# qinzheng93/GeoTransformer

Hardware: NVIDIA H100
Metric: point-cloud pairs/sec (3DMatch-shape synth) (higher is better)
Workload: dtype f32

## Files before the change

geotransformer_b200/csrc/evaluation.cu:

```cuda
#include "common.cuh"
#include "geob200.h"

namespace geob200 {

__device__ __forceinline__ float sqn3(float x, float y, float z) { return __fadd_rn(__fadd_rn(__fmul_rn(x, x), __fmul_rn(y, y)), __fmul_rn(z, z)); }
__device__ __forceinline__ float sqd_mm(float ax, float ay, float az, float a2, float bx, float by, float bz, float b2) {
    const float xy = fmaf(az, bz, fmaf(ay, by, __fmul_rn(ax, bx)));
    return fmaxf(__fadd_rn(__fsub_rn(a2, __fmul_rn(2.0f, xy)), b2), 0.0f);
}
__device__ __forceinline__ void xform(const float* T, float x, float y, float z, float& ox, float& oy, float& oz) {
    ox = fmaf(z, T[2], fmaf(y, T[1], x * T[0])) + T[3];
    oy = fmaf(z, T[6], fmaf(y, T[5], x * T[4])) + T[7];
    oz = fmaf(z, T[10], fmaf(y, T[9], x * T[8])) + T[11];
}

__global__ void __launch_bounds__(256) nc_prepare_kernel(const float* __restrict__ ref_nodes, const float* __restrict__ src_nodes,
                                                         const float* __restrict__ ref_knn_pts, const float* __restrict__ src_knn_pts,
                                                         const unsigned char* __restrict__ ref_knn_masks,
                                                         const unsigned char* __restrict__ src_knn_masks, const __grid_constant__ Segs cl,
                                                         int B, int K, const float* __restrict__ T, float* __restrict__ nodes_out,
                                                         float* __restrict__ pts_out, float* __restrict__ max_dist, int* __restrict__ n_valid) {
    const int lane = threadIdx.x & 31;
    const int s = blockIdx.y;
    const int m = blockIdx.x * 8 + (threadIdx.x >> 5);
    if (m >= cl.count[s]) return;
    const bool src = s >= B;
    const float* __restrict__ nodes = src ? src_nodes : ref_nodes;
    const float* __restrict__ knn_pts = src ? src_knn_pts : ref_knn_pts;
    const unsigned char* __restrict__ knn_masks = src ? src_knn_masks : ref_knn_masks;
    {
        const long long r = cl.start[s], r_in = src ? r - cl.start[B] : r;
        nodes += 3 * r_in; knn_pts += 3 * r_in * K; nodes_out += 3 * r; pts_out += 3 * r * K; max_dist += r; n_valid += r;
        if (knn_masks != nullptr) knn_masks += r_in * K;
        T = (T != nullptr && src) ? T + 16 * (s - B) : nullptr;
    }
    float nx = nodes[3 * m], ny = nodes[3 * m + 1], nz = nodes[3 * m + 2];
    if (T != nullptr) xform(T, nx, ny, nz, nx, ny, nz);
    float md = 0.f;
    int nv = 0;
    for (int i = lane; i < K; i += 32) {
        const float* p = knn_pts + ((long long)m * K + i) * 3;
        float px = p[0], py = p[1], pz = p[2];
        if (T != nullptr) xform(T, px, py, pz, px, py, pz);
        float* o = pts_out + ((long long)m * K + i) * 3;
        o[0] = px; o[1] = py; o[2] = pz;
        const bool ok = knn_masks == nullptr || knn_masks[(long long)m * K + i];
        const float dx = px - nx, dy = py - ny, dz = pz - nz;
        if (ok) { md = fmaxf(md, sqrtf(sqn3(dx, dy, dz))); ++nv; }
    }
    md = warp_max(md);
#pragma unroll
    for (int o = 16; o > 0; o >>= 1) nv += __shfl_xor_sync(0xffffffffu, nv, o);
    if (lane == 0) {
        nodes_out[3 * m] = nx; nodes_out[3 * m + 1] = ny; nodes_out[3 * m + 2] = nz;
        max_dist[m] = md;
        n_valid[m] = nv;
    }
}

__global__ void __launch_bounds__(256) nc_overlap_kernel(const float* __restrict__ ref_nodes, const float* __restrict__ src_nodes,
                                                         const float* __restrict__ ref_pts, const float* __restrict__ src_pts,
                                                         const unsigned char* __restrict__ ref_knn_masks,
                                                         const unsigned char* __restrict__ src_knn_masks,
                                                         const unsigned char* __restrict__ ref_masks, const unsigned char* __restrict__ src_masks,
                                                         const float* __restrict__ ref_max, const float* __restrict__ src_max,
                                                         const int* __restrict__ ref_nv, const int* __restrict__ src_nv,
                                                         const __grid_constant__ Segs R, const __grid_constant__ Segs Q,
                                                         const __grid_constant__ Segs NN, int K, float pos_radius,
                                                         float* __restrict__ overlap ) {
    const int b = blockIdx.y;
    const int M = R.count[b], N = Q.count[b];
    if ((int)blockIdx.x >= M) return;
    {
        const long long r = R.start[b], q = Q.start[b];
        ref_nodes += 3 * r; ref_pts += 3 * r * K; ref_max += r; ref_nv += r;
        if (ref_knn_masks != nullptr) ref_knn_masks += r * K;
        if (ref_masks != nullptr) ref_masks += r;
        src_nodes += 3 * q; src_pts += 3 * q * K; src_max += q; src_nv += q;
        if (src_knn_masks != nullptr) src_knn_masks += q * K;
        if (src_masks != nullptr) src_masks += q;
        overlap += NN.start[b];
    }
    extern __shared__ float sm[];
    float4* rp = reinterpret_cast<float4*>(sm);
    float4* sp = rp + K;
    int* rhit = reinterpret_cast<int*>(sp + K);
    int* shit = rhit + K;
    __shared__ int tot[2];
    const int m = blockIdx.x;
    const float r2 = pos_radius * pos_radius;
    for (int i = threadIdx.x; i < K; i += blockDim.x) {
        const float* p = ref_pts + ((long long)m * K + i) * 3;
        const bool ok = ref_knn_masks == nullptr || ref_knn_masks[(long long)m * K + i];
        rp[i] = make_float4(p[0], p[1], p[2], ok ? sqn3(p[0], p[1], p[2]) : -1.f);
    }
    const bool m_ok = ref_masks == nullptr || ref_masks[m];
    const float mx = ref_nodes[3 * m], my = ref_nodes[3 * m + 1], mz = ref_nodes[3 * m + 2];
    const float m2 = sqn3(mx, my, mz);
    __syncthreads();
    for (int n = 0; n < N; ++n) {
        float ov = 0.f;
        const bool n_ok = src_masks == nullptr || src_masks[n];
        const float sx = src_nodes[3 * n], sy = src_nodes[3 * n + 1], sz = src_nodes[3 * n + 2];
        const float dist = sqrtf(sqd_mm(mx, my, mz, m2, sx, sy, sz, sqn3(sx, sy, sz)));
        const bool inter = m_ok && n_ok && (ref_max[m] + src_max[n] + pos_radius - dist > 0.f);
        if (inter) {
            for (int j = threadIdx.x; j < K; j += blockDim.x) {
                const float* p = src_pts + ((long long)n * K + j) * 3;
                const bool ok = src_knn_masks == nullptr || src_knn_masks[(long long)n * K + j];
                sp[j] = make_float4(p[0], p[1], p[2], ok ? sqn3(p[0], p[1], p[2]) : -1.f);
                shit[j] = 0;
                rhit[j] = 0;
            }
            __syncthreads();
            for (int e = threadIdx.x; e < K * K; e += blockDim.x) {
                const int i = e / K, j = e % K;
                const float4 a = rp[i], b = sp[j];
                if (a.w >= 0.f && b.w >= 0.f && sqd_mm(a.x, a.y, a.z, a.w, b.x, b.y, b.z, b.w) < r2) { rhit[i] = 1; shit[j] = 1; }
            }
            __syncthreads();
            int cr = 0, cs = 0;
            for (int i = threadIdx.x; i < K; i += blockDim.x) { cr += rhit[i]; cs += shit[i]; }
            if (threadIdx.x == 0) { tot[0] = 0; tot[1] = 0; }
            __syncthreads();
            if (cr) atomicAdd(&tot[0], cr);
            if (cs) atomicAdd(&tot[1], cs);
            __syncthreads();
            ov = ((float)tot[0] / (float)ref_nv[m] + (float)tot[1] / (float)src_nv[n]) / 2.0f;
            __syncthreads();
        }
        if (threadIdx.x == 0) overlap[(long long)m * N + n] = ov;
    }
}

__global__ void __launch_bounds__(1024) nc_compact_kernel(const float* __restrict__ overlap, const __grid_constant__ Segs R,
                                                          const __grid_constant__ Segs Q, const __grid_constant__ Segs NN,
                                                          long long* __restrict__ idx, float* __restrict__ ov_out, int* __restrict__ count) {
    const int b = blockIdx.x;
    const int M = R.count[b], N = Q.count[b];
    overlap += NN.start[b]; idx += 2ll * NN.start[b]; ov_out += NN.start[b]; count += b;
    __shared__ int warp_tot[32];
    __shared__ int carry;
    const int lane = threadIdx.x & 31, warp = threadIdx.x >> 5;
    if (threadIdx.x == 0) carry = 0;
    __syncthreads();
    const long long total = (long long)M * N;
    for (long long base = 0; base < total; base += 4096) {
        const long long t0 = base + 4ll * threadIdx.x;
        float v[4];
        int f = 0;
#pragma unroll
        for (int u = 0; u < 4; ++u) {
            v[u] = (t0 + u < total) ? overlap[t0 + u] : 0.f;
            f += v[u] > 0.f ? 1 : 0;
        }
        int incl = f;
#pragma unroll
        for (int o = 1; o < 32; o <<= 1) {
            const int y = __shfl_up_sync(0xffffffffu, incl, o);
            if (lane >= o) incl += y;
        }
        if (lane == 31) warp_tot[warp] = incl;
        __syncthreads();
        int off = carry + incl - f;
        for (int w = 0; w < warp; ++w) off += warp_tot[w];
#pragma unroll
        for (int u = 0; u < 4; ++u)
            if (v[u] > 0.f) {
                idx[2ll * off] = (t0 + u) / N;
                idx[2ll * off + 1] = (t0 + u) % N;
                ov_out[off] = v[u];
                ++off;
            }
        __syncthreads();
        if (threadIdx.x == 0) { int s = 0; for (int w = 0; w < 32; ++w) s += warp_tot[w]; carry += s; }
        __syncthreads();
    }
    if (threadIdx.x == 0) *count = carry;
}

__global__ void __launch_bounds__(1024) evaluate_kernel(const long long* __restrict__ gt_idx, const float* __restrict__ gt_ov,
                                                        const __grid_constant__ Segs G, float acc_overlap,
                                                        const long long* __restrict__ ref_corr_idx, const long long* __restrict__ src_corr_idx,
                                                        int n_node_corr, const float* __restrict__ ref_corr_pts,
                                                        const float* __restrict__ src_corr_pts, int n_corr, float acc_radius,
                                                        const float* __restrict__ T_gt, const float* __restrict__ T_est, int t_ld,
                                                        const float* __restrict__ src_points, const __grid_constant__ Segs S0, int mode,
                                                        float acc_rmse, float acc_rre, float acc_rte, float* __restrict__ metrics, int m_ld,
                                                        const int* __restrict__ n_gt_dev, const int* __restrict__ n_node_corr_dev,
                                                        const int* __restrict__ n_corr_dev) {
    const int b = blockIdx.x;
    int n_gt = G.count[b];
    gt_idx += 2ll * G.start[b]; gt_ov += G.start[b];
    ref_corr_idx += (long long)b * n_node_corr; src_corr_idx += (long long)b * n_node_corr;
    ref_corr_pts += 3ll * b * n_corr; src_corr_pts += 3ll * b * n_corr;
    T_gt += 16 * b; T_est += (long long)b * t_ld;
    src_points += 3ll * S0.start[b];
    const int n_src = S0.count[b];
    metrics += (long long)b * m_ld;
    if (n_gt_dev != nullptr) n_gt_dev += b;
    if (n_node_corr_dev != nullptr) n_node_corr_dev += b;
    if (n_corr_dev != nullptr) n_corr_dev += b;
    if (n_gt_dev != nullptr) n_gt = *n_gt_dev;
    if (n_node_corr_dev != nullptr) n_node_corr = min(n_node_corr, *n_node_corr_dev);
    if (n_corr_dev != nullptr) n_corr = *n_corr_dev;
    __shared__ double red[32];
    __shared__ float Tg[16], Te[16], Tr[16];
    const int lane = threadIdx.x & 31, warp = threadIdx.x >> 5;
    if (threadIdx.x < 16) { Tg[threadIdx.x] = T_gt[threadIdx.x]; Te[threadIdx.x] = T_est[threadIdx.x]; }
    __syncthreads();
    auto block_sum = [&](double v) -> double {
        v = warp_sum_d(v);
        __syncthreads();
        if (lane == 0) red[warp] = v;
        __syncthreads();
        double s = 0.0;
        for (int w = 0; w < (int)(blockDim.x >> 5); ++w) s += red[w];
        return s;
    };
    const double nan = __longlong_as_double(0x7ff8000000000000LL);
    double hit = 0.0;
    for (int c = warp; c < n_node_corr; c += (int)(blockDim.x >> 5)) {
        const long long r = ref_corr_idx[c], s = src_corr_idx[c];
        int found = 0;
        for (int g = lane; g < n_gt; g += 32)
            if (gt_idx[2ll * g] == r && gt_idx[2ll * g + 1] == s && gt_ov[g] > acc_overlap) found = 1;
        found = __any_sync(0xffffffffu, found);
        if (lane == 0) hit += found;
    }
    const double hits = block_sum(hit);
    const double pir = n_node_corr > 0 ? hits / n_node_corr : nan;
    double inl = 0.0;
    for (int c = threadIdx.x; c < n_corr; c += blockDim.x) {
        float x, y, z;
        xform(Tg, src_corr_pts[3ll * c], src_corr_pts[3ll * c + 1], src_corr_pts[3ll * c + 2], x, y, z);
        const float dx = ref_corr_pts[3ll * c] - x, dy = ref_corr_pts[3ll * c + 1] - y, dz = ref_corr_pts[3ll * c + 2] - z;
        inl += (sqrtf(sqn3(dx, dy, dz)) < acc_radius) ? 1.0 : 0.0;
    }
    const double inls = block_sum(inl);
    const double ir = n_corr > 0 ? inls / n_corr : nan;
    if (threadIdx.x == 0) {
        for (int i = 0; i < 3; ++i) {
            for (int j = 0; j < 3; ++j) {
                double a = 0.0;
                for (int k = 0; k < 3; ++k) a += (double)Tg[4 * k + i] * Te[4 * k + j];
                Tr[4 * i + j] = (float)a;
            }
            double b = 0.0;
            for (int k = 0; k < 3; ++k) b += (double)Tg[4 * k + i] * ((double)Te[4 * k + 3] - Tg[4 * k + 3]);
            Tr[4 * i + 3] = (float)b;
        }
    }
    __syncthreads();
    double se = 0.0;
    if (mode != 1) {
        for (int p = threadIdx.x; p < n_src; p += blockDim.x) {
            const float px = src_points[3ll * p], py = src_points[3ll * p + 1], pz = src_points[3ll * p + 2];
            float x, y, z, gx = px, gy = py, gz = pz;
            if (mode == 0) {
                xform(Tr, px, py, pz, x, y, z);
            } else {
                xform(Te, px, py, pz, x, y, z);
                xform(Tg, px, py, pz, gx, gy, gz);
            }
            se += sqrtf(sqn3(x - gx, y - gy, z - gz));
        }
    }
    const double ses = block_sum(se);
    const double rmse = mode == 1 ? nan : (n_src > 0 ? ses / n_src : nan);
    if (threadIdx.x == 0) {
        float tr = 0.f;
        for (int i = 0; i < 3; ++i) {
            float d = 0.f;
            for (int k = 0; k < 3; ++k) d = fmaf(Te[4 * k + i], Tg[4 * k + i], d);
            tr += d;
        }
        float x = 0.5f * (tr - 1.0f);
        x = fminf(fmaxf(x, -1.0f), 1.0f);
        const float rre = 180.0f * acosf(x) / 3.14159265358979323846f;
        const float dtx = Tg[3] - Te[3], dty = Tg[7] - Te[7], dtz = Tg[11] - Te[11];
        const float rte = sqrtf(sqn3(dtx, dty, dtz));
        metrics[0] = (float)pir;
        metrics[1] = (float)ir;
        metrics[2] = rre;
// ... 197 lines not shown
        float s = 0.f;
        for (int k = 0; k < n; ++k) s += G[side ? (long long)k * N + line : (long long)line * N + k] * other[(long long)k * C + c];
        out[c] = s;
    }
}

__global__ void __launch_bounds__(32) closs_finalize_kernel(const float* __restrict__ ell_r, const unsigned char* __restrict__ kept_r,
                                                            const float* __restrict__ ell_c, const unsigned char* __restrict__ kept_c,
                                                            const __grid_constant__ Segs R, const __grid_constant__ Segs Q,
                                                            float* __restrict__ out, long long ld) {
    const int p = blockIdx.x, lane = threadIdx.x;
    double m[2];
    for (int side = 0; side < 2; ++side) {
        const float* ell = side ? ell_c : ell_r;
        const unsigned char* kept = side ? kept_c : kept_r;
        const int s0 = side ? Q.start[p] : R.start[p], n = side ? Q.count[p] : R.count[p];
        double s = 0.0, k = 0.0;
        for (int i = lane; i < n; i += 32)
            if (kept[s0 + i]) { s += ell[s0 + i]; k += 1.0; }
        s = warp_sum_d(s);
        k = warp_sum_d(k);
        m[side] = (float)(s / k);
    }
    if (lane == 0) out[p * ld + 1] = __fdiv_rn(__fadd_rn((float)m[0], (float)m[1]), 2.0f);
}

template <int K, int MODE>
__global__ void __launch_bounds__(256) floss_patch_kernel(const float* __restrict__ ref_pts, const float* __restrict__ src_pts,
                                                          const unsigned char* __restrict__ ref_masks,
                                                          const unsigned char* __restrict__ src_masks, float* __restrict__ scores,
                                                          const float* __restrict__ T, int P, const int* __restrict__ count, float r2,
                                                          double* __restrict__ psum, int* __restrict__ pcnt, const float* __restrict__ grad,
                                                          long long gld, int with_w, float w_f) {
    __shared__ float4 rp[K], sp[K];
    __shared__ int rhit[K], shit[K];
    __shared__ double redd[8];
    __shared__ int redi[8];
    __shared__ float Tm[16];
    const int p = blockIdx.y, q = blockIdx.x;
    const long long patch = (long long)p * P + q;
    const bool live = count == nullptr || q < count[p];
    if (threadIdx.x < 16) Tm[threadIdx.x] = T[16 * p + threadIdx.x];
    __syncthreads();
    for (int i = threadIdx.x; i < K; i += blockDim.x) {
        const float* a = ref_pts + (patch * K + i) * 3;
        const float* b = src_pts + (patch * K + i) * 3;
        const bool ra = live && ref_masks[patch * K + i], sa = live && src_masks[patch * K + i];
        float x, y, z;
        xform(Tm, b[0], b[1], b[2], x, y, z);
        rp[i] = make_float4(a[0], a[1], a[2], ra ? sqn3(a[0], a[1], a[2]) : -1.f);
        sp[i] = make_float4(x, y, z, sa ? sqn3(x, y, z) : -1.f);
        rhit[i] = 0;
        shit[i] = 0;
    }
    __syncthreads();
    float* S = scores + patch * (K + 1) * (K + 1);
    double s = 0.0;
    int n = 0;
    auto hit = [&](int i, int j) {
        const float4 a = rp[i], b = sp[j];
        return a.w >= 0.f && b.w >= 0.f && sqd_mm(a.x, a.y, a.z, a.w, b.x, b.y, b.z, b.w) < r2;
    };
    for (int e = threadIdx.x; e < K * K; e += blockDim.x) {
        const int i = e / K, j = e % K;
        if (hit(i, j)) {
            rhit[i] = 1;
            shit[j] = 1;
            if (MODE == 0) s += S[i * (K + 1) + j];
            ++n;
        }
    }
    __syncthreads();
    if constexpr (MODE == 2) {
        int np = 0;
        for (int k = threadIdx.x; k < P; k += blockDim.x) np += pcnt[(long long)p * P + k];
        np = block_reduce_256(np, [](int x, int y) { return x + y; }, redi);
        const float g = with_w ? grad[p * gld + 2] + w_f * grad[p * gld] : grad[p * gld + 2];
        const float val = np > 0 ? -g / (float)np : 0.f;
        for (int e = threadIdx.x; e < (K + 1) * (K + 1); e += blockDim.x) {
            const int i = e / (K + 1), j = e % (K + 1);
            bool lab;
            if (i < K && j < K) lab = hit(i, j);
            else if (i < K && j == K) lab = rp[i].w >= 0.f && !rhit[i];
            else if (i == K && j < K) lab = sp[j].w >= 0.f && !shit[j];
            else lab = false;
            S[e] = lab ? val : 0.f;
        }
    } else {
        for (int i = threadIdx.x; i < K; i += blockDim.x) {
            if (rp[i].w >= 0.f && !rhit[i]) { if (MODE == 0) s += S[i * (K + 1) + K]; ++n; }
            if (sp[i].w >= 0.f && !shit[i]) { if (MODE == 0) s += S[K * (K + 1) + i]; ++n; }
        }
        if (MODE == 0) s = block_reduce_256(s, [](double x, double y) { return x + y; }, redd);
        n = block_reduce_256(n, [](int x, int y) { return x + y; }, redi);
        if (threadIdx.x == 0) {
            if (MODE == 0) psum[patch] = s;
            pcnt[patch] = n;
        }
    }
}

__global__ void __launch_bounds__(32) floss_finalize_kernel(const double* __restrict__ psum, const int* __restrict__ pcnt, int P,
                                                            int with_total, float w_c, float w_f, float* __restrict__ out, long long ld) {
    const int p = blockIdx.x, lane = threadIdx.x;
    double s = 0.0, k = 0.0;
    for (int q = lane; q < P; q += 32) { s += psum[(long long)p * P + q]; k += pcnt[(long long)p * P + q]; }
    s = warp_sum_d(s);
    k = warp_sum_d(k);
    if (lane == 0) {
        const float f = -(float)(s / k);
        out[p * ld + 2] = f;
        if (with_total) out[p * ld] = __fadd_rn(__fmul_rn(w_c, out[p * ld + 1]), __fmul_rn(w_f, f));
    }
}

}

using namespace geob200;

extern "C" {

size_t geob200_node_correspondences_batched_workspace_bytes(int64_t n_rows, int64_t n_products, int64_t k) {
    const size_t r = (size_t)n_rows;
    return align_up(12 * r, 256) + align_up(12 * r * (size_t)k, 256) + 2 * align_up(4 * r, 256) + align_up(4 * (size_t)n_products, 256) + 256;
}

int geob200_node_correspondences_batched(const float* ref_nodes, const float* src_nodes, const float* ref_knn_points,
                                         const float* src_knn_points, const uint8_t* ref_masks, const uint8_t* src_masks,
                                         const uint8_t* ref_knn_masks, const uint8_t* src_knn_masks, int64_t n_pairs, const int64_t* cloud_nodes,
                                         int64_t k, const float* transforms, float pos_radius, int64_t* corr_indices, float* corr_overlaps,
                                         int32_t* count, void* workspace, size_t workspace_bytes, void* stream) {
    cudaStream_t st = (cudaStream_t)stream;
    GEOB_REQUIRE(n_pairs > 0 && 2 * n_pairs <= GEOB_MAX_CLOUDS, "node_correspondences_batched: 1..%d pairs", GEOB_MAX_CLOUDS / 2);
    GEOB_REQUIRE(k > 0 && k <= 1024, "node_correspondences: bad shape");
    const int B = (int)n_pairs;
    Segs cl, Q, NN;
    if (segs_from_counts(&cl, 2 * n_pairs, cloud_nodes) || segs_from_counts(&Q, n_pairs, cloud_nodes + n_pairs)) return -1;
    const Segs R = segs_range(cl, 0, B);
    const int64_t ref_rows = cl.start[B], rows = (int64_t)cl.start[2 * B - 1] + cl.count[2 * B - 1];
    GEOB_REQUIRE(ref_rows > 0 && rows > ref_rows, "node_correspondences: bad shape");
    if (segs_products(&NN, R, Q)) return -1;
    const int64_t nn = (int64_t)NN.start[B - 1] + NN.count[B - 1];
    GEOB_REQUIRE(workspace_bytes >= geob200_node_correspondences_batched_workspace_bytes(rows, nn, k),
                 "node_correspondences_batched: workspace too small");
    Arena ar(workspace, workspace_bytes);
    float* cn = ar.take<float>(3 * rows);
    float* cp = ar.take<float>(3 * rows * k);
    float* cmax = ar.take<float>(rows);
    int* cnv = ar.take<int>(rows);
    float* overlap = ar.take<float>(nn);
    GEOB_REQUIRE(ar.ok(), "node_correspondences: workspace accounting error");
    nc_prepare_kernel<<<dim3((unsigned)((cl.max + 7) / 8 > 0 ? (cl.max + 7) / 8 : 1), 2 * B), 256, 0, st>>>(
        ref_nodes, src_nodes, ref_knn_points, src_knn_points, ref_knn_masks, src_knn_masks, cl, B, (int)k, transforms, cn, cp, cmax, cnv);
    const size_t smem = (size_t)k * (2 * sizeof(float4) + 2 * sizeof(int));
    if (R.max > 0)
        nc_overlap_kernel<<<dim3((unsigned)R.max, B), 256, smem, st>>>(cn, cn + 3 * ref_rows, cp, cp + 3 * ref_rows * k, ref_knn_masks,
                                                                      src_knn_masks, ref_masks, src_masks, cmax, cmax + ref_rows, cnv,
                                                                      cnv + ref_rows, R, Q, NN, (int)k, pos_radius, overlap);
    nc_compact_kernel<<<B, 1024, 0, st>>>(overlap, R, Q, NN, (long long*)corr_indices, corr_overlaps, count);
    GEOB_CHECK_LAUNCH();
    count_launches(3);
    return 0;
}

static int evaluate_impl(const int64_t* gt_idx, const float* gt_ov, const Segs& G, const int32_t* n_gt_dev, float acceptance_overlap,
                         const int64_t* ref_idx, const int64_t* src_idx, int64_t n_node_corr, const int32_t* n_node_corr_dev,
                         const float* ref_pts, const float* src_pts, int64_t n_corr, const int32_t* n_corr_dev, float acceptance_radius,
                         const float* gt_transform, const float* est_transform, int64_t transform_ld, const float* src_points,
                         const Segs& S0, int mode, float rmse_threshold, float rre_threshold, float rte_threshold, float* metrics,
                         int64_t metrics_ld, cudaStream_t st) {
    GEOB_REQUIRE(mode >= 0 && mode <= 2, "evaluate: mode must be 0 (3DMatch), 1 (KITTI) or 2 (ModelNet)");
    evaluate_kernel<<<G.n, 1024, 0, st>>>((const long long*)gt_idx, gt_ov, G, acceptance_overlap, (const long long*)ref_idx,
                                          (const long long*)src_idx, (int)n_node_corr, ref_pts, src_pts, (int)n_corr, acceptance_radius,
                                          gt_transform, est_transform, (int)transform_ld, src_points, S0, mode, rmse_threshold, rre_threshold,
                                          rte_threshold, metrics, (int)metrics_ld, n_gt_dev, n_node_corr_dev, n_corr_dev);
    GEOB_CHECK_LAUNCH();
    count_launches(1);
    return 0;
}

int geob200_evaluate_counts(const int64_t* gt_node_corr_indices, const float* gt_node_corr_overlaps, int64_t n_gt, const int32_t* n_gt_dev,
                            float acceptance_overlap, const int64_t* ref_node_corr_indices, const int64_t* src_node_corr_indices,
                            int64_t n_node_corr, const int32_t* n_node_corr_dev, const float* ref_corr_points, const float* src_corr_points,
                            int64_t n_corr, const int32_t* n_corr_dev, float acceptance_radius, const float* gt_transform,
                            const float* est_transform, const float* src_points, int64_t n_src_points, int mode, float rmse_threshold,
                            float rre_threshold, float rte_threshold, float* metrics, void* stream) {
    return evaluate_impl(gt_node_corr_indices, gt_node_corr_overlaps, segs_one(n_gt), n_gt_dev, acceptance_overlap, ref_node_corr_indices,
                         src_node_corr_indices, n_node_corr, n_node_corr_dev, ref_corr_points, src_corr_points, n_corr, n_corr_dev,
                         acceptance_radius, gt_transform, est_transform, 16, src_points, segs_one(n_src_points), mode, rmse_threshold,
                         rre_threshold, rte_threshold, metrics, 8, (cudaStream_t)stream);
}

int geob200_evaluate_batched(const int64_t* gt_node_corr_indices, const float* gt_node_corr_overlaps, const int32_t* n_gt_dev,
                             float acceptance_overlap, const int64_t* ref_node_corr_indices, const int64_t* src_node_corr_indices,
                             int64_t n_node_corr, const int32_t* n_node_corr_dev, const float* ref_corr_points, const float* src_corr_points,
                             int64_t n_corr, const int32_t* n_corr_dev, float acceptance_radius, const float* gt_transforms,
                             const float* est_transforms, int64_t transform_ld, const float* points, int64_t n_pairs, const int64_t* cloud_nodes,
                             const int64_t* cloud_points, int mode, float rmse_threshold, float rre_threshold, float rte_threshold,
                             float* metrics, int64_t metrics_ld, void* stream) {
    GEOB_REQUIRE(n_pairs > 0 && 2 * n_pairs <= GEOB_MAX_CLOUDS, "evaluate_batched: 1..%d pairs", GEOB_MAX_CLOUDS / 2);
    GEOB_REQUIRE(transform_ld >= 16 && metrics_ld >= 8, "evaluate_batched: transform_ld >= 16 and metrics_ld >= 8 required");
    Segs cl, pt, G;
    if (segs_from_counts(&cl, 2 * n_pairs, cloud_nodes) || segs_from_counts(&pt, 2 * n_pairs, cloud_points)) return -1;
    const int B = (int)n_pairs;
    if (segs_products(&G, segs_range(cl, 0, B), segs_range(cl, B, B))) return -1;
    return evaluate_impl(gt_node_corr_indices, gt_node_corr_overlaps, G, n_gt_dev, acceptance_overlap, ref_node_corr_indices,
                         src_node_corr_indices, n_node_corr, n_node_corr_dev, ref_corr_points, src_corr_points, n_corr, n_corr_dev,
                         acceptance_radius, gt_transforms, est_transforms, transform_ld, points, segs_range(pt, B, B), mode, rmse_threshold,
                         rre_threshold, rte_threshold, metrics, metrics_ld, (cudaStream_t)stream);
}

size_t geob200_coarse_matching_loss_batched_workspace_bytes(int64_t n_rows, int64_t n_products) {
    const size_t r = (size_t)n_rows, nn = (size_t)n_products;
    return 2 * align_up(4 * nn, 256) + align_up(4 * r, 256) + align_up(r, 256) + 256;
}

int geob200_coarse_matching_loss_batched(const float* ref_feats, const float* src_feats, int64_t channels, int64_t n_pairs,
                                         const int64_t* cloud_nodes, const int64_t* gt_node_corr_indices, const float* gt_node_corr_overlaps,
                                         const int32_t* gt_count, float positive_margin, float negative_margin, float positive_optimal,
                                         float negative_optimal, float log_scale, float positive_overlap, float* out, int64_t out_ld,
                                         void* workspace, size_t workspace_bytes, void* stream) {
    cudaStream_t st = (cudaStream_t)stream;
    GEOB_REQUIRE(n_pairs > 0 && 2 * n_pairs <= GEOB_MAX_CLOUDS, "coarse_matching_loss_batched: 1..%d pairs", GEOB_MAX_CLOUDS / 2);
    GEOB_REQUIRE(channels > 0 && channels <= 8192, "coarse_matching_loss_batched: 1..8192 channels");
    GEOB_REQUIRE(log_scale > 0.f, "coarse_matching_loss_batched: log_scale must be positive");
    GEOB_REQUIRE(out_ld >= 3, "coarse_matching_loss_batched: out_ld >= 3 required");
    GEOB_REQUIRE(gt_count != nullptr, "coarse_matching_loss_batched: gt_count (device int32, one per pair) is required");
    for (int64_t c = 0; c < 2 * n_pairs; ++c) GEOB_REQUIRE(cloud_nodes[c] >= 0, "coarse_matching_loss_batched: negative node count");
    const int B = (int)n_pairs;
    Segs R, Q, NN;
    if (segs_from_counts(&R, B, cloud_nodes) || segs_from_counts(&Q, B, cloud_nodes + B) || segs_products(&NN, R, Q)) return -1;
    const int64_t rows = (int64_t)R.start[B - 1] + R.count[B - 1] + Q.start[B - 1] + Q.count[B - 1];
    const int64_t nn = (int64_t)NN.start[B - 1] + NN.count[B - 1];
    GEOB_REQUIRE(workspace_bytes >= geob200_coarse_matching_loss_batched_workspace_bytes(rows, nn),
                 "coarse_matching_loss_batched: workspace too small");
    Arena ar(workspace, workspace_bytes);
    float* d = ar.take<float>(nn);
    float* o = ar.take<float>(nn);
    float* ell = ar.take<float>(rows);
    unsigned char* kept = ar.take<unsigned char>(rows);
    GEOB_REQUIRE(ar.ok(), "coarse_matching_loss_batched: workspace accounting error");
    float* ell_c = ell + R.start[B - 1] + R.count[B - 1];
    unsigned char* kept_c = kept + R.start[B - 1] + R.count[B - 1];
    const CircleParams cp{positive_margin, negative_margin, positive_optimal, negative_optimal, log_scale, positive_overlap};
    int n_launch = 1;
    if (R.max > 0 && Q.max > 0) {
        closs_dist_kernel<<<dim3((unsigned)R.max, B), 256, channels * sizeof(float), st>>>(ref_feats, src_feats, (int)channels, R, Q, NN, d, o,
                                                                                           nullptr);
        closs_scatter_kernel<<<dim3((unsigned)((NN.max + 255) / 256), B), 256, 0, st>>>((const long long*)gt_node_corr_indices,
                                                                                        gt_node_corr_overlaps, gt_count, R, Q, NN, o);
        n_launch += 2;
    }
    if (R.max > 0 || Q.max > 0) {
        closs_lse_kernel<<<dim3((unsigned)(R.max > Q.max ? R.max : Q.max), B, 2), 256, 0, st>>>(d, o, R, Q, NN, cp, ell, kept, ell_c, kept_c,
                                                                                                nullptr, nullptr);
        n_launch += 1;
    }
    closs_finalize_kernel<<<B, 32, 0, st>>>(ell, kept, ell_c, kept_c, R, Q, out, (long long)out_ld);
    GEOB_CHECK_LAUNCH();
    count_launches(n_launch);
    return 0;
}

size_t geob200_fine_matching_loss_batched_workspace_bytes(int64_t n_pairs, int64_t n_patches) {
    const size_t n = (size_t)n_pairs * (size_t)n_patches;
    return align_up(8 * n, 256) + align_up(4 * n, 256) + 256;
}

int geob200_fine_matching_loss_batched(const float* ref_knn_points, const float* src_knn_points, const uint8_t* ref_knn_masks,
                                       const uint8_t* src_knn_masks, const float* matching_scores, const float* transforms, int64_t n_pairs,
                                       int64_t n_patches, int64_t k, const int32_t* patch_count, double positive_radius,
                                       const float* loss_weights, float* out, int64_t out_ld, void* workspace, size_t workspace_bytes,
                                       void* stream) {
    cudaStream_t st = (cudaStream_t)stream;
    GEOB_REQUIRE(n_pairs > 0 && n_pairs <= 65535, "fine_matching_loss_batched: 1..65535 pairs");
    GEOB_REQUIRE(n_patches >= 0 && n_patches < (1 << 30), "fine_matching_loss_batched: negative patch count");
    GEOB_REQUIRE(k == 64 || k == 128, "fine_matching_loss_batched: k must be 64 or 128, got %lld", (long long)k);
    GEOB_REQUIRE(positive_radius > 0.0, "fine_matching_loss_batched: positive_radius must be positive");
    GEOB_REQUIRE(out_ld >= 3, "fine_matching_loss_batched: out_ld >= 3 required");
    GEOB_REQUIRE(workspace_bytes >= geob200_fine_matching_loss_batched_workspace_bytes(n_pairs, n_patches),
                 "fine_matching_loss_batched: workspace too small");
    Arena ar(workspace, workspace_bytes);
    double* psum = ar.take<double>((size_t)n_pairs * n_patches);
    int* pcnt = ar.take<int>((size_t)n_pairs * n_patches);
    GEOB_REQUIRE(ar.ok(), "fine_matching_loss_batched: workspace accounting error");
    const float r2 = (float)(positive_radius * positive_radius);
    const int P = (int)n_patches;
    float w_c = 0.f, w_f = 0.f;
    if (loss_weights != nullptr) { w_c = loss_weights[0]; w_f = loss_weights[1]; }
    int n_launch = 1;
    if (P > 0) {
        const dim3 grid((unsigned)P, (unsigned)n_pairs);
        if (k == 64)
            floss_patch_kernel<64, 0><<<grid, 256, 0, st>>>(ref_knn_points, src_knn_points, ref_knn_masks, src_knn_masks,
                                                            const_cast<float*>(matching_scores), transforms, P, patch_count, r2, psum, pcnt,
                                                            nullptr, 0, 0, 0.f);
        else
            floss_patch_kernel<128, 0><<<grid, 256, 0, st>>>(ref_knn_points, src_knn_points, ref_knn_masks, src_knn_masks,
                                                             const_cast<float*>(matching_scores), transforms, P, patch_count, r2, psum, pcnt,
                                                             nullptr, 0, 0, 0.f);
        n_launch += 1;
    }
    floss_finalize_kernel<<<(unsigned)n_pairs, 32, 0, st>>>(psum, pcnt, P, loss_weights != nullptr, w_c, w_f, out, (long long)out_ld);
    GEOB_CHECK_LAUNCH();
    count_launches(n_launch);
    return 0;
}
// ... 103 lines not shown
```

geotransformer_b200/csrc/linear_tc.cu:

```cuda
#include <cuda.h>

#include <cstdlib>
#include <mutex>
#include <vector>

#include "common.cuh"
#include "geob200.h"
#include "hopper.cuh"

namespace geob200 {
namespace ltc {

using namespace hop;

constexpr int BM = 128;
constexpr int KC = 32;
constexpr int TILE_A = BM * 128;
constexpr int TILE_B = 128 * 128;
constexpr int STAGE = TILE_A + 2 * TILE_B;
constexpr int NSTAGE = 4;
constexpr int PRODUCER_WARP = 8;
constexpr int NTHREADS = (PRODUCER_WARP + 4) * 32;
constexpr int SMEM = NSTAGE * STAGE + 1024 + 256 + 8 * 128 * 8 + 512;

__global__ void __launch_bounds__(256) split_tf32_kernel(const float* __restrict__ w, long long ld, long long n, long long k,
                                                         float* __restrict__ out) {
    const long long nk = n * k;
    for (long long i = (long long)blockIdx.x * blockDim.x + threadIdx.x; i < nk; i += (long long)gridDim.x * blockDim.x) {
        const long long r = i / k, c = i % k;
        const float x = w[r * ld + c];
        const float hi = tf32_rn(x);
        out[i] = hi;
        out[nk + i] = x - hi;
    }
}

template <int BNI>
__global__ void __launch_bounds__(NTHREADS, 1) linear_tc_kernel(const __grid_constant__ CUtensorMap map_x,
                                                                const __grid_constant__ CUtensorMap map_w,
                                                                const float* __restrict__ bias, const float* __restrict__ row_scale,
                                                                float* __restrict__ Y, int ldy, int M, int N, int K, int BN, int relu,
                                                                GnFuse gn, float* __restrict__ splitk_out, int chunks_per_split,
                                                                int col_tiles, int row_tiles, int num_tiles) {
    constexpr int R = BNI / 2;
    extern __shared__ unsigned char smem_raw[];
    unsigned char* smem = (unsigned char*)(((uintptr_t)smem_raw + 1023) & ~(uintptr_t)1023);
    uint64_t* bars = (uint64_t*)(smem + NSTAGE * STAGE);
    uint64_t* full = bars;
    uint64_t* empty = bars + NSTAGE;
    float2* gn_sm = (float2*)(smem + NSTAGE * STAGE + 256);
    float* bias_s = (float*)(gn_sm + 8 * 128);
    const int warp = threadIdx.x >> 5, lane = threadIdx.x & 31;
    const int nk = (K + KC - 1) / KC;
    const int tiles_per_split = col_tiles * row_tiles;

    if (threadIdx.x == 0) {
        for (int s = 0; s < NSTAGE; ++s) { mbar_init(&full[s], 1); mbar_init(&empty[s], 8); }
        asm volatile("fence.mbarrier_init.release.cluster;" ::: "memory");
        asm volatile("prefetch.tensormap [%0];" ::"l"(&map_x) : "memory");
        asm volatile("prefetch.tensormap [%0];" ::"l"(&map_w) : "memory");
    }
    __syncthreads();

    if (warp >= PRODUCER_WARP) {
        asm volatile("setmaxnreg.dec.sync.aligned.u32 40;" ::: "memory");
        if (warp == PRODUCER_WARP && lane == 0) {
            int s = 0;
            uint32_t ph = 0;
            for (int t = blockIdx.x; t < num_tiles; t += gridDim.x) {
                const int z = t / tiles_per_split, rem = t % tiles_per_split;
                const int m0 = (rem / col_tiles) * BM, n0 = (rem % col_tiles) * BN;
                const int kc0 = z * chunks_per_split, kc1 = min(nk, kc0 + chunks_per_split);
                for (int kc = kc0; kc < kc1; ++kc) {
                    mbar_wait(&empty[s], ph ^ 1u);
                    unsigned char* st = smem + s * STAGE;
                    mbar_arrive_expect_tx(&full[s], (uint32_t)(TILE_A + 2 * BN * 128));
                    tma_load_2d(st, &map_x, kc * KC, m0, &full[s]);
                    tma_load_2d(st + TILE_A, &map_w, kc * KC, n0, &full[s]);
                    tma_load_2d(st + TILE_A + TILE_B, &map_w, kc * KC, N + n0, &full[s]);
                    if (++s == NSTAGE) { s = 0; ph ^= 1u; }
                }
            }
        }
        return;
    }

    asm volatile("setmaxnreg.inc.sync.aligned.u32 232;" ::: "memory");
    const int wg = warp >> 2, wq = warp & 3;
    int s = 0;
    uint32_t ph = 0;
    for (int t = blockIdx.x; t < num_tiles; t += gridDim.x) {
        const int z = t / tiles_per_split, rem = t % tiles_per_split;
        const int ty = rem / col_tiles;
        const int m0 = ty * BM, n0 = (rem % col_tiles) * BN;
        const int kc0 = z * chunks_per_split, kc1 = min(nk, kc0 + chunks_per_split);
        asm volatile("bar.sync 1, 256;" ::: "memory");
        if (threadIdx.x < 128) bias_s[threadIdx.x] = (bias != nullptr && (int)threadIdx.x < BN) ? __ldg(bias + n0 + threadIdx.x) : 0.f;
        asm volatile("bar.sync 1, 256;" ::: "memory");

        float acc[R], cor[R];
#pragma unroll
        for (int i = 0; i < R; ++i) { acc[i] = 0.f; cor[i] = 0.f; }
        const int g = lane >> 2, tq = lane & 3;
        const int a_off = (wg * 64 + wq * 16 + g) * 128 + tq * 4;
        for (int kc = kc0; kc < kc1; ++kc) {
            mbar_wait(&full[s], ph);
            unsigned char* st = smem + s * STAGE;
            uint32_t f[2][KC / 8][4];
#pragma unroll
            for (int kk = 0; kk < KC / 8; ++kk)
#pragma unroll
                for (int e = 0; e < 4; ++e) {
                    const int j = 2 * kk + (e >> 1);
                    const float x = *reinterpret_cast<const float*>(st + a_off + (e & 1) * 8 * 128 + ((j ^ g) << 4));
                    const float hi = tf32_rn(x);
                    f[0][kk][e] = __float_as_uint(hi);
                    f[1][kk][e] = __float_as_uint(x - hi);
                }
            const uint32_t sb = smem_u32(st + TILE_A);
            const uint64_t b_hi = make_desc(sb), b_lo = make_desc(sb + TILE_B);
            wgmma_fence();
#pragma unroll
            for (int kk = 0; kk < KC / 8; ++kk) {
                const uint64_t adv = (uint64_t)(kk * 2);
                const uint32_t accum = (kc == kc0 && kk == 0) ? 0u : 1u;
                wgmma_tf32_rs<BNI>(acc, f[0][kk], b_hi + adv, accum);
                wgmma_tf32_rs<BNI>(cor, f[0][kk], b_lo + adv, accum);
                wgmma_tf32_rs<BNI>(cor, f[1][kk], b_hi + adv, 1u);
            }
            wgmma_commit();
            wgmma_wait<0>();
            __syncwarp();
            if (lane == 0) mbar_arrive(&empty[s]);
            if (++s == NSTAGE) { s = 0; ph ^= 1u; }
        }
        reg_fence(acc);
        reg_fence(cor);

        const int r0 = m0 + wg * 64 + wq * 16 + (lane >> 2);
        const int c0 = 2 * (lane & 3);
        float rs[2];
#pragma unroll
        for (int h = 0; h < 2; ++h) rs[h] = (row_scale != nullptr && r0 + 8 * h < M) ? row_scale[r0 + 8 * h] : 1.0f;
        if (splitk_out != nullptr) {
#pragma unroll
            for (int j = 0; j < BNI / 8; ++j)
#pragma unroll
                for (int h = 0; h < 2; ++h) {
                    const int m = r0 + 8 * h, col = 8 * j + c0;
                    if (m < M && col < BN)
                        *reinterpret_cast<float2*>(splitk_out + ((long long)z * M + m) * N + n0 + col) =
                            make_float2(acc[4 * j + 2 * h] + cor[4 * j + 2 * h], acc[4 * j + 2 * h + 1] + cor[4 * j + 2 * h + 1]);
                }
            continue;
        }
        const bool vec2 = ((ldy & 1) == 0) && ((reinterpret_cast<uintptr_t>(Y) & 7) == 0);
#pragma unroll
        for (int j = 0; j < BNI / 8; ++j) {
            const int col = 8 * j + c0;
            float o[4];
#pragma unroll
            for (int e = 0; e < 4; ++e) {
                float v = (acc[4 * j + e] + cor[4 * j + e]) * rs[e >> 1] + bias_s[col + (e & 1)];
                if (relu) v = fmaxf(v, 0.f);
                o[e] = v;
            }
#pragma unroll
            for (int h = 0; h < 2; ++h) {
                const int m = r0 + 8 * h;
                if (m < M && col < BN) {
                    float* yp = Y + (long long)m * ldy + n0 + col;
                    if (vec2) *reinterpret_cast<float2*>(yp) = make_float2(o[2 * h], o[2 * h + 1]);
                    else { yp[0] = o[2 * h]; yp[1] = o[2 * h + 1]; }
                }
            }
            if (gn.groups > 0) {
                const bool ok0 = r0 < M && col < BN, ok1 = r0 + 8 < M && col < BN;
                float a0 = (ok0 ? o[0] : 0.f) + (ok1 ? o[2] : 0.f), a1 = (ok0 ? o[1] : 0.f) + (ok1 ? o[3] : 0.f);
                float q0 = (ok0 ? o[0] * o[0] : 0.f) + (ok1 ? o[2] * o[2] : 0.f);
                float q1 = (ok0 ? o[1] * o[1] : 0.f) + (ok1 ? o[3] * o[3] : 0.f);
#pragma unroll
                for (int off = 4; off < 32; off <<= 1) {
                    a0 += __shfl_xor_sync(0xffffffffu, a0, off);
                    a1 += __shfl_xor_sync(0xffffffffu, a1, off);
                    q0 += __shfl_xor_sync(0xffffffffu, q0, off);
                    q1 += __shfl_xor_sync(0xffffffffu, q1, off);
                }
                if (lane < 4) {
                    gn_sm[warp * 128 + col] = make_float2(a0, q0);
                    gn_sm[warp * 128 + col + 1] = make_float2(a1, q1);
                }
            }
        }
        if (gn.groups > 0) {
            asm volatile("bar.sync 1, 256;" ::: "memory");
            const int sw = gn.slot_width, slots_tile = BN / sw, slots_total = N / sw;
            const int et = threadIdx.x;
            if (et < slots_tile) {
                double s1 = 0.0, s2 = 0.0;
                for (int w = 0; w < 8; ++w) {
                    float f1 = 0.f, f2 = 0.f;
                    for (int c = 0; c < sw; ++c) {
                        const float2 p = gn_sm[w * 128 + et * sw + c];
                        f1 += p.x;
                        f2 += p.y;
                    }
                    s1 += (double)f1;
                    s2 += (double)f2;
                }
                double* dst = gn.partial + ((long long)ty * slots_total + n0 / sw + et) * 2;
                dst[0] = s1;
                dst[1] = s2;
            }
        }
    }
}

__global__ void __launch_bounds__(256) splitk_reduce_kernel(const float* __restrict__ P, int splits, long long MN, int N,
                                                            const float* __restrict__ bias, const float* __restrict__ row_scale,
                                                            float* __restrict__ Y, int ldy, int relu) {
    const long long i4 = ((long long)blockIdx.x * blockDim.x + threadIdx.x) * 4;
    if (i4 >= MN) return;
    float4 a = *reinterpret_cast<const float4*>(P + i4);
    for (int z = 1; z < splits; ++z) {
        const float4 b = *reinterpret_cast<const float4*>(P + (long long)z * MN + i4);
        a.x += b.x; a.y += b.y; a.z += b.z; a.w += b.w;
    }
    const long long m = i4 / N;
    const int n = (int)(i4 % N);
    const float rs = row_scale != nullptr ? row_scale[m] : 1.0f;
    float o[4] = {a.x * rs, a.y * rs, a.z * rs, a.w * rs};
#pragma unroll
    for (int u = 0; u < 4; ++u) {
        if (bias != nullptr) o[u] += bias[n + u];
        if (relu) o[u] = fmaxf(o[u], 0.f);
    }
    float* y = Y + m * ldy + n;
    if ((reinterpret_cast<uintptr_t>(y) & 15) == 0) *reinterpret_cast<float4*>(y) = make_float4(o[0], o[1], o[2], o[3]);
    else { y[0] = o[0]; y[1] = o[1]; y[2] = o[2]; y[3] = o[3]; }
}

typedef CUresult (*EncodeTiledFn)(CUtensorMap*, CUtensorMapDataType, cuuint32_t, void*, const cuuint64_t*, const cuuint64_t*,
                                  const cuuint32_t*, const cuuint32_t*, CUtensorMapInterleave, CUtensorMapSwizzle,
                                  CUtensorMapL2promotion, CUtensorMapFloatOOBfill);
static EncodeTiledFn encode_fn() {
    static EncodeTiledFn fn = nullptr;
    if (fn == nullptr) {
        void* p = nullptr;
        cudaDriverEntryPointQueryResult q;
        if (cudaGetDriverEntryPoint("cuTensorMapEncodeTiled", &p, cudaEnableDefault, &q) == cudaSuccess && q == cudaDriverEntryPointSuccess)
            fn = (EncodeTiledFn)p;
    }
    return fn;
}

static int encode_map(CUtensorMap* map, const float* base, int64_t rows, int64_t cols, int64_t ld, int box_rows) {
    EncodeTiledFn fn = encode_fn();
    if (fn == nullptr) { set_error("cuTensorMapEncodeTiled entry point not available"); return -1; }
    cuuint64_t gdim[2] = {(cuuint64_t)cols, (cuuint64_t)rows};
    cuuint64_t gstride[1] = {(cuuint64_t)ld * sizeof(float)};
    cuuint32_t box[2] = {(cuuint32_t)KC, (cuuint32_t)box_rows};
    cuuint32_t estr[2] = {1, 1};
    CUresult r = fn(map, CU_TENSOR_MAP_DATA_TYPE_FLOAT32, 2, (void*)base, gdim, gstride, box, estr, CU_TENSOR_MAP_INTERLEAVE_NONE,
                    CU_TENSOR_MAP_SWIZZLE_128B, CU_TENSOR_MAP_L2_PROMOTION_L2_128B, CU_TENSOR_MAP_FLOAT_OOB_FILL_NONE);
    if (r != CUDA_SUCCESS) { set_error("cuTensorMapEncodeTiled failed with CUresult %d", (int)r); return -1; }
    return 0;
}

}

struct ProfRec { cudaEvent_t a, b; long long m, n, k; };
static std::vector<ProfRec> g_prof;
static std::mutex g_prof_mu;
static bool g_prof_on = false;
static bool g_splitk_on = true;
static bool g_persistent_on = true;

struct StreamWs { void* ptr; size_t bytes; };
static std::vector<std::pair<cudaStream_t, StreamWs>> g_split_ws, g_wimg_ws;
static std::mutex g_split_mu;
static float* stream_scratch(std::vector<std::pair<cudaStream_t, StreamWs>>& pool, cudaStream_t st, size_t bytes) {
    std::lock_guard<std::mutex> lk(g_split_mu);
    for (auto& e : pool)
        if (e.first == st) {
            if (e.second.bytes >= bytes) return (float*)e.second.ptr;
            cudaFreeAsync(e.second.ptr, st);
            e.second = {nullptr, 0};
            if (cudaMallocAsync(&e.second.ptr, bytes * 2, st) != cudaSuccess) return nullptr;
            e.second.bytes = bytes * 2;
            return (float*)e.second.ptr;
        }
    StreamWs w{nullptr, 0};
    const size_t cap = bytes * 2 > (16u << 20) ? bytes * 2 : (16u << 20);
    if (cudaMallocAsync(&w.ptr, cap, st) != cudaSuccess) return nullptr;
    w.bytes = cap;
    pool.push_back({st, w});
    return (float*)w.ptr;
}

static void launch_split_tf32(const float* w, int64_t ld, int64_t n, int64_t k, float* out, cudaStream_t st) {
    const long long nk = (long long)n * k;
    long long blocks = (nk + 255) / 256;
    if (blocks > 4LL * num_sms()) blocks = 4LL * num_sms();
    ltc::split_tf32_kernel<<<(unsigned)(blocks > 0 ? blocks : 1), 256, 0, st>>>(w, ld, n, k, out);
    count_launches(1);
}

int linear_tc(const float* x, int64_t ldx, const float* w, int64_t ldw, const float* w_img, const float* bias, const float* row_scale,
              float* y, int64_t ldy, int64_t m, int64_t n, int64_t k, int relu, cudaStream_t st, const GnFuse* gn) {
    if (m < 64 || n < 32 || (n % 16) != 0 || (k % 4) != 0 || (ldx % 4) != 0) return 1;
    if ((reinterpret_cast<uintptr_t>(x) & 15) || (reinterpret_cast<uintptr_t>(w_img) & 15)) return 1;
    if (w_img == nullptr && ((ldw % 4) != 0 || (reinterpret_cast<uintptr_t>(w) & 15))) return 1;
    if (n > 128 && (n % 128) != 0) return 1;
    const int BN = (int)(n >= 128 ? 128 : n);
    const int col_tiles = (int)(n / BN), row_tiles = (int)((m + ltc::BM - 1) / ltc::BM);
    GnFuse g{};
    if (gn != nullptr) {
        g = *gn;
        const int64_t cpg = n / g.groups;
        if (g.groups <= 0 || n % g.groups != 0 || (cpg < 32 ? (32 % cpg) != 0 : (cpg % 32) != 0 || (BN % cpg) != 0) || relu) return 1;
        g.slot_width = (int)(cpg < 32 ? cpg : 32);
    }
    const int nk = (int)((k + ltc::KC - 1) / ltc::KC);
    const int tiles = col_tiles * row_tiles;
    int splits = 1;
    if (g_splitk_on && tiles * 2 <= num_sms() && nk >= 16) {
        splits = nk / 8;
        if (splits > num_sms() / tiles) splits = num_sms() / tiles;
        if (splits > 16) splits = 16;
        if (splits < 2) splits = 1;
    }
    if (gn != nullptr && splits > 1) return 1;
    int cps = nk;
    float* part = nullptr;
    if (splits > 1) {
        cps = (nk + splits - 1) / splits;
        splits = (nk + cps - 1) / cps;
        part = stream_scratch(g_split_ws, st, (size_t)splits * (size_t)m * (size_t)n * sizeof(float));
        if (part == nullptr) { splits = 1; cps = nk; }
    }
    float* img = nullptr;
    if (w_img == nullptr) {
        img = stream_scratch(g_wimg_ws, st, (size_t)2 * (size_t)n * (size_t)k * sizeof(float));
        if (img == nullptr) { set_error("linear_tc: weight image scratch allocation failed"); return -1; }
        w_img = img;
    }
    CUtensorMap mx, mw;
    if (ltc::encode_map(&mx, x, m, k, ldx, ltc::BM)) return -1;
    if (ltc::encode_map(&mw, w_img, 2 * n, k, k, BN)) return -1;
    ProfRec rec{};
    const bool prof = g_prof_on;
    if (prof) {
        cudaEventCreate(&rec.a);
        cudaEventCreate(&rec.b);
        rec.m = m; rec.n = n; rec.k = k;
        cudaEventRecord(rec.a, st);
    }
    if (img != nullptr) launch_split_tf32(w, ldw, n, k, img, st);
    const int num_tiles = tiles * splits;
    const bool persistent = g_persistent_on && splits == 1 && tiles > num_sms();
    const unsigned grid = (unsigned)(persistent ? num_sms() : num_tiles);
    const void* kern = BN <= 32 ? (const void*)ltc::linear_tc_kernel<32> : BN <= 64 ? (const void*)ltc::linear_tc_kernel<64>
                                                                                      : (const void*)ltc::linear_tc_kernel<128>;
    if (ensure_max_smem(kern)) return -1;
#define GEOB_LTC_LAUNCH(BNI)                                                                                                  \
    ltc::linear_tc_kernel<BNI><<<grid, ltc::NTHREADS, ltc::SMEM, st>>>(mx, mw, bias, row_scale, y, (int)ldy, (int)m, (int)n, (int)k, \
                                                                       BN, relu, g, part, cps, col_tiles, row_tiles, num_tiles)
    if (BN <= 32) GEOB_LTC_LAUNCH(32);
    else if (BN <= 64) GEOB_LTC_LAUNCH(64);
    else GEOB_LTC_LAUNCH(128);
#undef GEOB_LTC_LAUNCH
    if (part != nullptr) {
        const long long mn = (long long)m * n;
        ltc::splitk_reduce_kernel<<<(unsigned)((mn / 4 + 255) / 256), 256, 0, st>>>(part, splits, mn, (int)n, bias, row_scale, y, (int)ldy, relu);
        count_launches(1);
    }
    if (prof) {
        cudaEventRecord(rec.b, st);
        std::lock_guard<std::mutex> lk(g_prof_mu);
        g_prof.push_back(rec);
    }
    GEOB_CHECK_LAUNCH();
    count_launches(1);
    return 0;
}

}

extern "C" {

int geob200_set_linear_persistent(int on) {
    geob200::g_persistent_on = on != 0;
    return 0;
}

int geob200_split_tf32(const float* w, int64_t ld, int64_t n, int64_t k, float* out, void* stream) {
    GEOB_REQUIRE(n > 0 && k > 0 && ld >= k, "split_tf32: bad shape (%lld x %lld, ld %lld)", (long long)n, (long long)k, (long long)ld);
    geob200::launch_split_tf32(w, ld, n, k, out, (cudaStream_t)stream);
    GEOB_CHECK_LAUNCH();
    return 0;
}

int geob200_set_split_k(int on) {
    geob200::g_splitk_on = on != 0;
    return 0;
}

int geob200_linear_profile_enable(int on) {
    std::lock_guard<std::mutex> lk(geob200::g_prof_mu);
    for (auto& r : geob200::g_prof) { cudaEventDestroy(r.a); cudaEventDestroy(r.b); }
    geob200::g_prof.clear();
    geob200::g_prof_on = on != 0;
    return 0;
}

int64_t geob200_linear_profile_read(int64_t capacity, int64_t* shapes, float* ms) {
    std::lock_guard<std::mutex> lk(geob200::g_prof_mu);
    int64_t n = 0;
    for (auto& r : geob200::g_prof) {
        if (n >= capacity) break;
        if (cudaEventSynchronize(r.b) != cudaSuccess) break;
        float t = 0.f;
        cudaEventElapsedTime(&t, r.a, r.b);
        shapes[3 * n] = r.m; shapes[3 * n + 1] = r.n; shapes[3 * n + 2] = r.k;
        ms[n] = t;
        ++n;
    }
    return n;
}

}
```

Baseline: 430.2.

## Assign one warp per source node in overlap kernel; size TMA ring per tile width

The node-overlap kernel now gives each warp its own source node instead of having the whole block walk source nodes serially. Each warp streams source points from registers, tests them against the shared reference points, and records hits as bitmasks reduced with warp intrinsics. This removes the many block-wide barriers and shared atomics that were paid per source node. Separately, the TF32 linear kernel now sizes its stage count from a fixed 192 KB ring for each BN template, so narrower tiles get deeper pipelines, which adds shared-memory and barrier-count constraints.

```diff
diff --git a/geotransformer_b200/csrc/evaluation.cu b/geotransformer_b200/csrc/evaluation.cu
--- a/geotransformer_b200/csrc/evaluation.cu
+++ b/geotransformer_b200/csrc/evaluation.cu
@@ -82,54 +82,65 @@
         overlap += NN.start[b];
     }
     extern __shared__ float sm[];
+    const int nw = (K + 31) / 32;
     float4* rp = reinterpret_cast<float4*>(sm);
-    float4* sp = rp + K;
-    int* rhit = reinterpret_cast<int*>(sp + K);
-    int* shit = rhit + K;
-    __shared__ int tot[2];
+    unsigned* rhit = reinterpret_cast<unsigned*>(rp + 32 * nw);
     const int m = blockIdx.x;
+    const int warp = threadIdx.x >> 5, lane = threadIdx.x & 31;
     const float r2 = pos_radius * pos_radius;
-    for (int i = threadIdx.x; i < K; i += blockDim.x) {
-        const float* p = ref_pts + ((long long)m * K + i) * 3;
-        const bool ok = ref_knn_masks == nullptr || ref_knn_masks[(long long)m * K + i];
-        rp[i] = make_float4(p[0], p[1], p[2], ok ? sqn3(p[0], p[1], p[2]) : -1.f);
+    for (int i = threadIdx.x; i < 32 * nw; i += blockDim.x) {
+        if (i < K) {
+            const float* p = ref_pts + ((long long)m * K + i) * 3;
+            const bool ok = ref_knn_masks == nullptr || ref_knn_masks[(long long)m * K + i];
+            rp[i] = make_float4(p[0], p[1], p[2], ok ? sqn3(p[0], p[1], p[2]) : -1.f);
+        } else {
+            rp[i] = make_float4(0.f, 0.f, 0.f, -1.f);
+        }
     }
     const bool m_ok = ref_masks == nullptr || ref_masks[m];
     const float mx = ref_nodes[3 * m], my = ref_nodes[3 * m + 1], mz = ref_nodes[3 * m + 2];
     const float m2 = sqn3(mx, my, mz);
     __syncthreads();
-    for (int n = 0; n < N; ++n) {
+    unsigned* rw = rhit + warp * nw;
+    for (int n = warp; n < N; n += blockDim.x >> 5) {
         float ov = 0.f;
         const bool n_ok = src_masks == nullptr || src_masks[n];
         const float sx = src_nodes[3 * n], sy = src_nodes[3 * n + 1], sz = src_nodes[3 * n + 2];
         const float dist = sqrtf(sqd_mm(mx, my, mz, m2, sx, sy, sz, sqn3(sx, sy, sz)));
         const bool inter = m_ok && n_ok && (ref_max[m] + src_max[n] + pos_radius - dist > 0.f);
         if (inter) {
-            for (int j = threadIdx.x; j < K; j += blockDim.x) {
-                const float* p = src_pts + ((long long)n * K + j) * 3;
-                const bool ok = src_knn_masks == nullptr || src_knn_masks[(long long)n * K + j];
-                sp[j] = make_float4(p[0], p[1], p[2], ok ? sqn3(p[0], p[1], p[2]) : -1.f);
-                shit[j] = 0;
-                rhit[j] = 0;
+            for (int w = lane; w < nw; w += 32) rw[w] = 0u;
+            __syncwarp();
+            int cs = 0;
+            for (int sb = 0; sb < nw; ++sb) {
+                const int j = 32 * sb + lane;
+                float4 b = make_float4(0.f, 0.f, 0.f, -1.f);
+                if (j < K) {
+                    const float* p = src_pts + ((long long)n * K + j) * 3;
+                    const bool ok = src_knn_masks == nullptr || src_knn_masks[(long long)n * K + j];
+                    b = make_float4(p[0], p[1], p[2], ok ? sqn3(p[0], p[1], p[2]) : -1.f);
+                }
+                bool hit_j = false;
+                for (int w = 0; w < nw; ++w) {
+                    unsigned bits = 0u;
+#pragma unroll 8
+                    for (int l = 0; l < 32; ++l) {
+                        const float4 a = rp[32 * w + l];
+                        if (a.w >= 0.f && b.w >= 0.f && sqd_mm(a.x, a.y, a.z, a.w, b.x, b.y, b.z, b.w) < r2) bits |= 1u << l;
+                    }
+                    hit_j = hit_j || bits != 0u;
+                    bits = __reduce_or_sync(0xffffffffu, bits);
+                    if (lane == 0) rw[w] |= bits;
+                }
+                cs += __popc(__ballot_sync(0xffffffffu, hit_j));
             }
-            __syncthreads();
-            for (int e = threadIdx.x; e < K * K; e += blockDim.x) {
-                const int i = e / K, j = e % K;
-                const float4 a = rp[i], b = sp[j];
-                if (a.w >= 0.f && b.w >= 0.f && sqd_mm(a.x, a.y, a.z, a.w, b.x, b.y, b.z, b.w) < r2) { rhit[i] = 1; shit[j] = 1; }
-            }
-            __syncthreads();
-            int cr = 0, cs = 0;
-            for (int i = threadIdx.x; i < K; i += blockDim.x) { cr += rhit[i]; cs += shit[i]; }
-            if (threadIdx.x == 0) { tot[0] = 0; tot[1] = 0; }
-            __syncthreads();
-            if (cr) atomicAdd(&tot[0], cr);
-            if (cs) atomicAdd(&tot[1], cs);
-            __syncthreads();
-            ov = ((float)tot[0] / (float)ref_nv[m] + (float)tot[1] / (float)src_nv[n]) / 2.0f;
-            __syncthreads();
-        }
-        if (threadIdx.x == 0) overlap[(long long)m * N + n] = ov;
+            __syncwarp();
+            int cr = 0;
+            for (int w = 0; w < nw; ++w) cr += __popc(rw[w]);
+            ov = ((float)cr / (float)ref_nv[m] + (float)cs / (float)src_nv[n]) / 2.0f;
+            __syncwarp();
+        }
+        if (lane == 0) overlap[(long long)m * N + n] = ov;
     }
 }
 
@@ -633,7 +644,7 @@
     GEOB_REQUIRE(ar.ok(), "node_correspondences: workspace accounting error");
     nc_prepare_kernel<<<dim3((unsigned)((cl.max + 7) / 8 > 0 ? (cl.max + 7) / 8 : 1), 2 * B), 256, 0, st>>>(
         ref_nodes, src_nodes, ref_knn_points, src_knn_points, ref_knn_masks, src_knn_masks, cl, B, (int)k, transforms, cn, cp, cmax, cnv);
-    const size_t smem = (size_t)k * (2 * sizeof(float4) + 2 * sizeof(int));
+    const size_t smem = (size_t)((k + 31) / 32) * (32 * sizeof(float4) + 8 * sizeof(unsigned));
     if (R.max > 0)
         nc_overlap_kernel<<<dim3((unsigned)R.max, B), 256, smem, st>>>(cn, cn + 3 * ref_rows, cp, cp + 3 * ref_rows * k, ref_knn_masks,
                                                                       src_knn_masks, ref_masks, src_masks, cmax, cmax + ref_rows, cnv,
diff --git a/geotransformer_b200/csrc/linear_tc.cu b/geotransformer_b200/csrc/linear_tc.cu
--- a/geotransformer_b200/csrc/linear_tc.cu
+++ b/geotransformer_b200/csrc/linear_tc.cu
@@ -15,13 +15,25 @@
 
 constexpr int BM = 128;
 constexpr int KC = 32;
-constexpr int TILE_A = BM * 128;
-constexpr int TILE_B = 128 * 128;
-constexpr int STAGE = TILE_A + 2 * TILE_B;
-constexpr int NSTAGE = 4;
+constexpr int ROW_BYTES = KC * (int)sizeof(float);
+static_assert(ROW_BYTES == 128, "SWIZZLE_128B rows hold 32 fp32 K values");
+constexpr int TILE_A = BM * ROW_BYTES;
+constexpr int RING_BYTES = 192 * 1024;
 constexpr int PRODUCER_WARP = 8;
 constexpr int NTHREADS = (PRODUCER_WARP + 4) * 32;
-constexpr int SMEM = NSTAGE * STAGE + 1024 + 256 + 8 * 128 * 8 + 512;
+
+template <int BNI>
+struct Cfg {
+    static constexpr int TILE_B = BNI * ROW_BYTES;
+    static constexpr int STAGE = TILE_A + 2 * TILE_B;
+    static constexpr int NSTAGE = RING_BYTES / STAGE;
+    static constexpr int SMEM = NSTAGE * STAGE + 1024 + 256 + 8 * 128 * 8 + 512;
+    static_assert(TILE_B % 1024 == 0 && STAGE % 1024 == 0, "SWIZZLE_128B operands start on 1024-byte boundaries");
+    static_assert(NSTAGE >= 4 && 2 * NSTAGE * 8 <= 256, "the full / empty barriers fit their 256 bytes");
+};
+__host__ __device__ constexpr uint32_t stage_tx_bytes(int bn) { return (uint32_t)(TILE_A + 2 * bn * ROW_BYTES); }
+static_assert(stage_tx_bytes(32) == Cfg<32>::STAGE && stage_tx_bytes(64) == Cfg<64>::STAGE && stage_tx_bytes(128) == Cfg<128>::STAGE,
+              "a tile of BNI columns fills its stage exactly");
 
 __global__ void __launch_bounds__(256) split_tf32_kernel(const float* __restrict__ w, long long ld, long long n, long long k,
                                                          float* __restrict__ out) {
@@ -43,6 +55,7 @@
                                                                 GnFuse gn, float* __restrict__ splitk_out, int chunks_per_split,
                                                                 int col_tiles, int row_tiles, int num_tiles) {
     constexpr int R = BNI / 2;
+    constexpr int NSTAGE = Cfg<BNI>::NSTAGE, STAGE = Cfg<BNI>::STAGE, TILE_B = Cfg<BNI>::TILE_B;
     extern __shared__ unsigned char smem_raw[];
     unsigned char* smem = (unsigned char*)(((uintptr_t)smem_raw + 1023) & ~(uintptr_t)1023);
     uint64_t* bars = (uint64_t*)(smem + NSTAGE * STAGE);
@@ -74,7 +87,7 @@
                 for (int kc = kc0; kc < kc1; ++kc) {
                     mbar_wait(&empty[s], ph ^ 1u);
                     unsigned char* st = smem + s * STAGE;
-                    mbar_arrive_expect_tx(&full[s], (uint32_t)(TILE_A + 2 * BN * 128));
+                    mbar_arrive_expect_tx(&full[s], stage_tx_bytes(BN));
                     tma_load_2d(st, &map_x, kc * KC, m0, &full[s]);
                     tma_load_2d(st + TILE_A, &map_w, kc * KC, n0, &full[s]);
                     tma_load_2d(st + TILE_A + TILE_B, &map_w, kc * KC, N + n0, &full[s]);
@@ -364,7 +377,7 @@
                                                                                       : (const void*)ltc::linear_tc_kernel<128>;
     if (ensure_max_smem(kern)) return -1;
 #define GEOB_LTC_LAUNCH(BNI)                                                                                                  \
-    ltc::linear_tc_kernel<BNI><<<grid, ltc::NTHREADS, ltc::SMEM, st>>>(mx, mw, bias, row_scale, y, (int)ldy, (int)m, (int)n, (int)k, \
+    ltc::linear_tc_kernel<BNI><<<grid, ltc::NTHREADS, ltc::Cfg<BNI>::SMEM, st>>>(mx, mw, bias, row_scale, y, (int)ldy, (int)m, (int)n, (int)k, \
                                                                        BN, relu, g, part, cps, col_tiles, row_tiles, num_tiles)
     if (BN <= 32) GEOB_LTC_LAUNCH(32);
     else if (BN <= 64) GEOB_LTC_LAUNCH(64);
```

Result: faster. 447.3, median of 6 (+4.0%).
